# djene-mengistu/UAPS

Hardware: AMD Instinct MI355X
Metric: training images/sec (labeled+unlabeled) NEU-Seg 256x256 K=3 (higher is better)
Workload: dtype f32

## Files before the change

include/uaps_hip.h:

```cpp
#ifndef UAPS_HIP_H
#define UAPS_HIP_H

#include <stddef.h>
#include <stdint.h>

#ifdef __cplusplus
extern "C" {
#endif

typedef void* uaps_stream_t;

#define UAPS_MAX_HEADS 8
#define UAPS_MAX_CLASSES 8

#define UAPS_OK 0
#define UAPS_EINVAL (-1)
#define UAPS_ERANGE (-2)
#define UAPS_EWORKSPACE (-3)
#define UAPS_ENOFORM (-4)

int uaps_abi_version(void);
const char* uaps_error_string(int code);


// ... 81 lines not shown
                        uint8_t* keep_out, uaps_stream_t stream);
int uaps_feat_mask_apply(const float* x, const uint8_t* keep, float scale, float* y, long n, uaps_stream_t stream);

int uaps_feat_dropout_workspace_bytes(int B, int C, int H, int W, size_t* out_host);
int uaps_feat_dropout_fwd(const float* x, float* y, int B, int C, int H, int W, float u, uint8_t* keep,
                          void* workspace, size_t workspace_bytes, uaps_stream_t stream);
int uaps_feat_dropout_bwd(const float* dy, const uint8_t* keep, float* dx, int B, int C, int H, int W,
                          uaps_stream_t stream);

int uaps_sum_tensors(const float* const* in_host, int n, float* out, long count, uaps_stream_t stream);
int uaps_fanin_perturbed(const float* const* g_host, const int* mode_host, const uint8_t* const* keep_host,
                         const uint64_t* offsets_host, int n, int groups, uint64_t seed, float range, float p, int B,
                         int C, int H, int W, float* out, uaps_stream_t stream);

int uaps_feat_dropout_stats(const float* x, int B, int C, int H, int W, void* workspace, size_t workspace_bytes,
                            uaps_stream_t stream);
int uaps_fanout_perturbed(const float* f, float* const* out_host, const int* mode_host, uint8_t* const* keep_host,
                          const uint64_t* offsets_host, const float* u_host, const void* fdrop_workspace, int n, int groups,
                          uint64_t seed, float range, float p, int B, int C, int H, int W, uaps_stream_t stream);

int uaps_maxpool2x2_fwd(const float* x, int B, int C, int H, int W, float* out, uint8_t* idx, uaps_stream_t stream);


int uaps_bn_workspace_bytes(int B, int C, int H, int W, size_t* out_host);
int uaps_bn_act_fwd_train(const float* y, const float* conv_bias, const float* gamma, const float* beta,
                          float* running_mean, float* running_var, int64_t* num_batches_tracked, float momentum,
                          float eps, float slope, float drop_p, uint64_t seed, uint64_t offset, int B, int C,
                          int H, int W, float* out, float* save_mean, float* save_invstd, void* workspace,
                          size_t workspace_bytes, uaps_stream_t stream);
int uaps_bn_act_fwd_train_grouped(const float* y, const float* conv_bias, const float* gamma, const float* beta,
                                  float* running_mean, float* running_var, int64_t* num_batches_tracked, float momentum,
                                  float eps, float slope, float drop_p, uint64_t seed, uint64_t offset, int B, int C,
                                  int H, int W, int groups, float* out, float* save_mean, float* save_invstd,
                                  void* workspace, size_t workspace_bytes, uaps_stream_t stream);
int uaps_bn_act_fwd_train_partials(const void* partials, int parts_per_image, const float* y, const float* conv_bias,
                                   const float* gamma, const float* beta, float* running_mean, float* running_var,
                                   int64_t* num_batches_tracked, float momentum, float eps, float slope, float drop_p,
                                   uint64_t seed, uint64_t offset, int B, int C, int H, int W, int groups, float* out,
                                   float* save_mean, float* save_invstd, void* workspace, size_t workspace_bytes,
                                   uaps_stream_t stream);
int uaps_bn_act_bwd_grouped(const float* dout, const float* y, const float* gamma, const float* beta,
                            const float* save_mean, const float* save_invstd, float slope, float drop_p, uint64_t seed,
                            uint64_t offset, int B, int C, int H, int W, int groups, float* dy, float* dgamma,
                            float* dbeta, void* workspace, size_t workspace_bytes, uaps_stream_t stream);
int uaps_bn_act_bwd_grouped_bias(const float* dout, const float* y, const float* gamma, const float* beta,
                                 const float* save_mean, const float* save_invstd, float slope, float drop_p,
                                 uint64_t seed, uint64_t offset, int B, int C, int H, int W, int groups, float* dy,
                                 float* dgamma, float* dbeta, float* dconv_bias, void* workspace, size_t workspace_bytes,
                                 uaps_stream_t stream);
int uaps_bn_act_fwd_eval(const float* y, const float* conv_bias, const float* gamma, const float* beta,
                         const float* running_mean, const float* running_var, float eps, float slope, int B,
                         int C, int H, int W, float* out, float* save_mean, void* workspace,
                         size_t workspace_bytes, uaps_stream_t stream);
int uaps_bn_act_bwd(const float* dout, const float* y, const float* gamma, const float* beta,
                    const float* save_mean, const float* save_invstd, float slope, float drop_p, uint64_t seed,
                    uint64_t offset, int B, int C, int H, int W, float* dy, float* dgamma, float* dbeta,
                    void* workspace, size_t workspace_bytes, uaps_stream_t stream);
int uaps_bn_act_bwd_eval(const float* dout, const float* y, const float* gamma, const float* beta,
                         const float* mean_eff, const float* running_var, float eps, float slope, int B, int C,
                         int H, int W, float* dy, void* workspace, size_t workspace_bytes, uaps_stream_t stream);

int uaps_up_cat_fwd(const float* skip, const float* low, float* out, int B, int Cs, int Cl, int h, int w,
                    uaps_stream_t stream);
int uaps_up_cat_bwd(const float* dout, float* dskip, float* dlow, int B, int Cs, int Cl, int h, int w,
                    uaps_stream_t stream);

int uaps_bn_param_bounds(const float* const* gamma_host, const float* const* beta_host, const int* C_host, int n, float* out,
                         uaps_stream_t stream);

int uaps_conv_set_mode(int mode);
#define UAPS_TUNE_NO_SPLIT_FWD 1u
#define UAPS_TUNE_NO_SPLIT_WRW 2u
#define UAPS_TUNE_NO_SMALL 4u
#define UAPS_TUNE_NO_HP16 8u
#define UAPS_TUNE_WRW_ROW_MAJOR 16u
#define UAPS_TUNE_WRW_SHORT_TILES 32u
#define UAPS_TUNE_NO_TALL_FWD 64u
#define UAPS_TUNE_NO_ROW16 128u
#define UAPS_TUNE_NO_ROW_WRW 256u
#define UAPS_TUNE_DEEP_ROWS 512u
#define UAPS_TUNE_G1_NARROW 1024u
#define UAPS_TUNE_NO_G 2048u
#define UAPS_TUNE_G_DEEP 4096u
int uaps_conv_set_tuning(unsigned flags);
unsigned uaps_conv_get_tuning(void);

#define UAPS_ERR_CONV_NONFINITE 1u
#define UAPS_ERR_WRW_NONFINITE 2u
int uaps_set_error_word(unsigned* device_word);

#define UAPS_BOUND_SLOTS 16
#define UAPS_BOUND_STRIDE 64
#define UAPS_BOUND_FLOATS (UAPS_BOUND_SLOTS * UAPS_BOUND_STRIDE)
typedef struct uaps_call_hints {
    unsigned struct_size;
    const float* bound[3];
    float mul[3];
    float* out_amax;
    const float* stats_mean;
    const float* stats_bias;
    const float* residual;
    const float* dyt_y;
    const float* dyt_coef;
    float* dyt_out;
    float dyt_slope;
    int dyt_groups;
    const float* bsum_y;
    const float* bsum_mean;
    const float* bsum_invstd;
    const float* bsum_gamma;
    const float* bsum_beta;
    void* bsum_partials;
    float* bsum_max;
    float bsum_slope;
    int bsum_groups;
} uaps_call_hints;
int uaps_next_call_hints(const uaps_call_hints* hints);
int uaps_next_launch_events(void* start, void* stop);
int uaps_account(int enable);
double uaps_accounted_bytes(void);
int uaps_zero_bounds(float* bounds, long n, uaps_stream_t stream);
int uaps_conv_get_mode(void);
int uaps_conv_pack_floats(int Cout, int Cin, int ks, size_t* fwd_floats_host, size_t* bwd_floats_host);
int uaps_conv_pack_weights(const float* w, int Cout, int Cin, int ks, float* wf, float* wb, uaps_stream_t stream);
int uaps_conv_pack_weights_batch(const float* const* w_host, float* const* wf_host, float* const* wb_host,
                                 const int* Cout_host, const int* Cin_host, const int* ks_host, int n,
                                 uaps_stream_t stream);
int uaps_conv_fwd(const float* x, const float* wf, const float* bias, float* y, int B, int Cin, int Cout, int H,
                  int W, int ks, int cfg, uaps_stream_t stream);
int uaps_conv_fwd_stats(const float* x, const float* wf, const float* bias, float* y, void* stats, int B, int Cin,
                        int Cout, int H, int W, int ks, int cfg, uaps_stream_t stream);
int uaps_conv_fwd_stats_parts(int B, int Cin, int Cout, int H, int W, int ks, int cfg, int* parts_per_image_host);
int uaps_conv_bwd_data(const float* dy, const float* wb, float* dx, int B, int Cin, int Cout, int H, int W,
                       int ks, int cfg, uaps_stream_t stream);
int uaps_conv_wrw_workspace_bytes(int B, int Cin, int Cout, int H, int W, int ks, int cfg, size_t* out_host);
int uaps_conv_bwd_weight_partial(const float* dy, const float* x, int want_bias, int B, int Cin, int Cout, int H, int W,
                                 int ks, int cfg, void* workspace, size_t workspace_bytes, uaps_stream_t stream);
int uaps_conv_bwd_weight_reduce(const void* workspace, float* dw, float* dbias, int B, int Cin, int Cout, int H, int W,
                                int ks, int cfg, uaps_stream_t stream);
typedef struct uaps_wrw_reduce_item {
    const void* workspace; float* dw; float* dbias;
    int B, Cin, Cout, H, W, ks, cfg;
} uaps_wrw_reduce_item;
int uaps_conv_bwd_weight_reduce_batch(const uaps_wrw_reduce_item* items, int n, uaps_stream_t stream);
#define UAPS_CONV_X2_UP2 (1 << 10)
#define UAPS_CONV_BOUNDED (1 << 11)
int uaps_conv_fwd_cat(const float* x1, int C1, const float* x2, int C2, const float* wf, const float* bias, float* y,
                      void* stats_or_null, int B, int Cout, int H, int W, int ks, int cfg, uaps_stream_t stream);
int uaps_conv_bwd_data_cat(const float* dy, const float* wb, float* dx1, int C1, float* dx2, int C2, int B, int Cout,
                           int H, int W, int ks, int cfg, uaps_stream_t stream);
int uaps_conv_bwd_weight_partial_cat(const float* dy, const float* x1, int C1, const float* x2, int C2, int want_bias,
                                     int B, int Cout, int H, int W, int ks, int cfg, void* workspace,
                                     size_t workspace_bytes, uaps_stream_t stream);
int uaps_bn_finalize_train(const void* partials, int parts_per_image, const float* conv_bias, const float* gamma,
                           const float* beta, float* running_mean, float* running_var, int64_t* num_batches_tracked,
                           float momentum, float eps, int B, int C, int H, int W, int groups, float* save_mean,
                           float* save_invstd, void* xf, uaps_stream_t stream);
int uaps_conv_fwd_bn(const float* x_raw, const void* xf, float slope, int groups, const float* wf, const float* bias,
                     float* y, void* stats_or_null, int B, int Cin, int Cout, int H, int W, int ks, int cfg,
                     uaps_stream_t stream);
int uaps_conv_bwd_weight_partial_bn(const float* dy, const float* x_raw, const void* xf, float slope, int groups,
                                    int want_bias, int B, int Cin, int Cout, int H, int W, int ks, int cfg,
                                    void* workspace, size_t workspace_bytes, uaps_stream_t stream);
#define UAPS_CONV_FWD 0
#define UAPS_CONV_BWD_DATA 1
#define UAPS_CONV_BWD_WEIGHT 2
// ... 165 lines not shown
```

uaps_amd/_lib.py:

```python
from __future__ import annotations

import ctypes as C
import os
import subprocess
import threading

from . import config

_HERE = os.path.dirname(os.path.abspath(__file__))
LIB_PATH = config.text("UAPS_HIP_LIB") or os.path.join(_HERE, "lib", "libuaps_hip.so")
CSRC = os.path.join(_HERE, "csrc")

_lock = threading.Lock()
_tls = threading.local()
_lib = None

c_float_p = C.POINTER(C.c_float)
c_void_p = C.c_void_p

_PTR = C.c_void_p
SIGNATURES = {
    "uaps_abi_version": (C.c_int, []),
    "uaps_error_string": (C.c_char_p, [C.c_int]),
    "uaps_loss_workspace_bytes": (C.c_int, [C.c_int] * 5 + [C.POINTER(C.c_size_t)]),
# ... 79 lines not shown
    "uaps_softmax_klmap_bwd": (C.c_int, [_PTR] * 3 + [C.c_int] * 4 + [_PTR] * 3),
    "uaps_softmax_pair_fwd": (C.c_int, [_PTR, _PTR] + [C.c_int] * 5 + [_PTR, _PTR, _PTR, _PTR, C.c_size_t, _PTR]),
    "uaps_softmax_mse_bwd": (C.c_int, [_PTR] * 3 + [C.c_int] * 4 + [_PTR, _PTR]),
    "uaps_softmax_kl_bwd": (C.c_int, [_PTR] * 3 + [C.c_int] * 4 + [_PTR, _PTR]),
    "uaps_entropy_map": (C.c_int, [_PTR] + [C.c_int] * 4 + [_PTR, _PTR, _PTR, C.c_size_t, _PTR]),
    "uaps_fanin_perturbed": (C.c_int, [_PTR] * 4 + [C.c_int, C.c_int, C.c_uint64, C.c_float, C.c_float] + [C.c_int] * 4 + [_PTR, _PTR]),
    "uaps_maxpool2x2_fwd": (C.c_int, [_PTR] + [C.c_int] * 4 + [_PTR, _PTR, _PTR]),
    "uaps_adam_step": (C.c_int, [_PTR] * 5 + [C.c_int] + [C.c_double] * 5 + [C.c_long, _PTR]),
    "uaps_add_relu": (C.c_int, [_PTR, _PTR, _PTR, C.c_long, _PTR]),
    "uaps_relu_bwd": (C.c_int, [_PTR, _PTR, _PTR, C.c_long, _PTR]),
    "uaps_relu_bwd_sum": (C.c_int, [_PTR, C.c_int, _PTR, _PTR, C.c_long, _PTR]),
    "uaps_cat2": (C.c_int, [_PTR, _PTR, _PTR, C.c_long, _PTR]),
    "uaps_bn_act_bwd_prepare": (C.c_int, [_PTR] * 6 + [C.c_float] + [C.c_int] * 5 + [_PTR] * 6 + [C.c_size_t, _PTR]),
    "uaps_bn_act_bwd_apply": (C.c_int, [_PTR] * 3 + [C.c_float] + [C.c_int] * 5 + [_PTR, _PTR]),
    "uaps_bn_act_bwd_finalize": (C.c_int, [_PTR, C.c_int] + [_PTR] * 5 + [C.c_int] * 5 + [_PTR] * 6),
    "uaps_seg_confusion": (C.c_int, [_PTR, _PTR] + [C.c_int] * 4 + [_PTR, _PTR]),
    "uaps_ema_update": (C.c_int, [_PTR] * 3 + [C.c_int, C.c_float, C.c_float, _PTR]),
    "uaps_teacher_noise": (C.c_int, [_PTR] + [C.c_int] * 5 + [C.c_uint64, C.c_uint64, _PTR, _PTR]),
    "uaps_teacher_noise_apply": (C.c_int, [_PTR, _PTR] + [C.c_int] * 5 + [_PTR, _PTR]),
    "uaps_mc_consistency_workspace_bytes": (C.c_int, [C.POINTER(C.c_size_t)]),
    "uaps_mc_consistency_fwd": (C.c_int, [_PTR] * 3 + [C.c_int] * 5 + [C.c_float] + [_PTR] * 4 + [C.c_size_t, _PTR]),
    "uaps_mc_consistency_bwd": (C.c_int, [_PTR] * 5 + [C.c_int] * 4 + [_PTR, _PTR]),
    "uaps_cct_dct_workspace_bytes": (C.c_int, [C.POINTER(C.c_size_t)]),
    "uaps_cct_consistency_fwd": (C.c_int, [_PTR] + [C.c_int] * 6 + [_PTR, _PTR, C.c_size_t, _PTR]),
    "uaps_cct_consistency_bwd": (C.c_int, [_PTR] + [C.c_int] * 6 + [_PTR, _PTR, _PTR]),
    "uaps_rot90_batch": (C.c_int, [_PTR, _PTR] + [C.c_int] * 5 + [_PTR, _PTR, _PTR]),
    "uaps_rot_consistency_fwd": (C.c_int, [_PTR, C.c_int, _PTR] + [C.c_int] * 6 + [_PTR, _PTR, C.c_size_t, _PTR]),
    "uaps_rot_consistency_bwd": (C.c_int, [_PTR, C.c_int, _PTR] + [C.c_int] * 6 + [_PTR, _PTR, _PTR, _PTR]),
    "uaps_cps_workspace_bytes": (C.c_int, [C.c_int] * 5 + [C.POINTER(C.c_size_t)]),
    "uaps_cps_fwd": (C.c_int, [_PTR] * 3 + [C.c_int] * 5 + [C.c_float] + [_PTR] * 4 + [C.c_size_t, _PTR]),
    "uaps_cps_bwd": (C.c_int, [_PTR] * 7 + [C.c_int] * 5 + [_PTR] * 3),
}


HINTED = ("uaps_conv_fwd", "uaps_conv_fwd_stats", "uaps_conv_fwd_bn", "uaps_conv_fwd_cat", "uaps_conv_bwd_data", "uaps_conv_bwd_data_cat",
          "uaps_conv_bwd_weight_partial", "uaps_conv_bwd_weight_partial_bn", "uaps_conv_bwd_weight_partial_cat",
          "uaps_bn_act_fwd_train_partials", "uaps_bn_finalize_train", "uaps_bn_act_bwd_grouped", "uaps_bn_act_bwd_grouped_bias",
          "uaps_bn_act_bwd_apply", "uaps_up_cat_fwd", "uaps_cat2", "uaps_add_relu", "uaps_pairloss_bwd", "uaps_rot90_batch")
for _n in HINTED:
    SIGNATURES[_n + "_h"] = (SIGNATURES[_n][0], [_PTR] + list(SIGNATURES[_n][1]))
del _n


class UapsHipError(RuntimeError):
    pass


def build(verbose: bool = False, jobs: int = 8) -> str:
    cmd = ["make", "-C", CSRC, f"-j{jobs}"]
    r = subprocess.run(cmd, stdout=subprocess.PIPE, stderr=subprocess.STDOUT, text=True)
    if verbose or r.returncode != 0:
        print(r.stdout)
    if r.returncode != 0:
        raise UapsHipError("building libuaps_hip.so failed (see output above)")
    return LIB_PATH


def lib() -> C.CDLL:
    global _lib
    if _lib is not None:
        return _lib
    with _lock:
        if _lib is None:
            if not os.path.exists(LIB_PATH):
                raise UapsHipError(
                    f"{LIB_PATH} not found: the UAPS HIP kernels are not built. Run "
                    "`make -C uaps_amd/csrc` (needs hipcc; cross-compiles for gfx950 without a GPU). "
                    "uaps_amd has no CPU or PyTorch fallback for these ops.")
            l = C.CDLL(LIB_PATH)
            for name, (res, args) in SIGNATURES.items():
                try:
                    fn = getattr(l, name)
                except AttributeError as e:
                    raise UapsHipError(f"libuaps_hip.so does not export {name}; rebuild it") from e
                fn.restype, fn.argtypes = res, args
            _configure_from_environment(l)
            _lib = l
    return _lib


_TUNE_ENV = (("UAPS_DIAG_NO_SPLIT_FWD", 1, None), ("UAPS_DIAG_NO_SPLIT_WRW", 2, None), ("UAPS_DIAG_NO_SMALL", 4, None),
             ("UAPS_DIAG_NO_HP16", 8, None), ("UAPS_SWRW_COLMAJOR", 16, "0"), ("UAPS_WRW_TALL", 32, "0"), ("UAPS_FWD_TALL", 64, "0"),
             ("UAPS_DIAG_NO_ROW16", 128, None), ("UAPS_DIAG_NO_ROW_WRW", 256, None), ("UAPS_DIAG_DEEP_ROWS", 512, None),
             ("UAPS_DIAG_G1_NARROW", 1024, None), ("UAPS_DIAG_NO_G", 2048, None), ("UAPS_DIAG_G_DEEP", 4096, None))


def _configure_from_environment(l) -> None:
    mode = config.text("UAPS_CONV_MODE")
    if mode:
        m = 0 if mode[0] in "0ef" else (1 if mode[0] in "1bs" else 2)
        if l.uaps_conv_set_mode(m) != 0:
            raise UapsHipError(f"UAPS_CONV_MODE={mode}: uaps_conv_set_mode failed")
    flags = 0
    for name, bit, on_value in _TUNE_ENV:
        v = config.text(name)
        if v is not None and (on_value is None or v == on_value):
            flags |= bit
    l.uaps_conv_set_tuning(flags)


class quiet_gc:

    def __enter__(self):
        import gc
        gc.collect()
        self.was = gc.isenabled()
        gc.disable()
        return self

    def __exit__(self, *exc):
        import gc
        if self.was:
            gc.enable()
        return False


class WrwReduceItem(C.Structure):
    _fields_ = [("workspace", C.c_void_p), ("dw", C.c_void_p), ("dbias", C.c_void_p), ("B", C.c_int), ("Cin", C.c_int), ("Cout", C.c_int),
                ("H", C.c_int), ("W", C.c_int), ("ks", C.c_int), ("cfg", C.c_int)]


class CallHints(C.Structure):
    _fields_ = [("struct_size", C.c_uint), ("bound", C.c_void_p * 3), ("mul", C.c_float * 3), ("out_amax", C.c_void_p),
                ("stats_mean", C.c_void_p), ("stats_bias", C.c_void_p), ("residual", C.c_void_p),
                ("dyt_y", C.c_void_p), ("dyt_coef", C.c_void_p), ("dyt_out", C.c_void_p), ("dyt_slope", C.c_float), ("dyt_groups", C.c_int),
                ("bsum_y", C.c_void_p), ("bsum_mean", C.c_void_p), ("bsum_invstd", C.c_void_p), ("bsum_gamma", C.c_void_p),
                ("bsum_beta", C.c_void_p), ("bsum_partials", C.c_void_p), ("bsum_max", C.c_void_p), ("bsum_slope", C.c_float),
                ("bsum_groups", C.c_int)]


class ConvCall(C.Structure):
    _fields_ = [("struct_size", C.c_uint), ("op", C.c_int), ("B", C.c_int), ("Cin", C.c_int), ("Cout", C.c_int), ("H", C.c_int),
                ("W", C.c_int), ("ks", C.c_int), ("cfg", C.c_int), ("x", C.c_void_p), ("C1", C.c_int), ("x2", C.c_void_p),
                ("w_packed", C.c_void_p), ("bias", C.c_void_p), ("y", C.c_void_p), ("y2", C.c_void_p), ("y_grad", C.c_void_p),
                ("stats", C.c_void_p), ("xf", C.c_void_p), ("xf_slope", C.c_float), ("xf_groups", C.c_int), ("want_bias", C.c_int),
                ("workspace", C.c_void_p), ("workspace_bytes", C.c_size_t), ("stream", C.c_void_p), ("hints", CallHints)]


def mk_hints(bounds=(), out_amax=None, stats=None, residual=None, dyt=None, bsum=None):
    h = getattr(_tls, "hints", None)
    if h is None:
        h = _tls.hints = CallHints()
        h.struct_size = C.sizeof(CallHints)
    for i in range(3):
        h.bound[i] = None
    h.out_amax = h.stats_mean = h.stats_bias = None
    h.residual = residual.data_ptr() if residual is not None else None
    if dyt is not None:
        h.dyt_y, h.dyt_coef, h.dyt_out, h.dyt_slope, h.dyt_groups = dyt[0].data_ptr(), dyt[1].data_ptr(), dyt[2].data_ptr(), float(dyt[3]), int(dyt[4])
    else:
        h.dyt_y = h.dyt_coef = h.dyt_out = None
        h.dyt_slope, h.dyt_groups = 0.0, 0
    if bsum is not None:
        (h.bsum_y, h.bsum_mean, h.bsum_invstd, h.bsum_gamma, h.bsum_beta, h.bsum_partials, h.bsum_max) = [t.data_ptr() for t in bsum[:7]]
        h.bsum_slope, h.bsum_groups = float(bsum[7]), int(bsum[8])
    else:
        h.bsum_y = h.bsum_mean = h.bsum_invstd = h.bsum_gamma = h.bsum_beta = h.bsum_partials = h.bsum_max = None
        h.bsum_slope, h.bsum_groups = 0.0, 0
    if stats is not None:
        if stats[0] is not None:
            h.stats_mean = stats[0].data_ptr()
        if stats[1] is not None:
            h.stats_bias = stats[1].data_ptr()
    for i, b in enumerate(bounds):
        if b is not None:
            h.bound[i], h.mul[i] = b[0].data_ptr(), float(b[1])
    if out_amax is not None:
# ... 103 lines not shown
```

uaps_amd/config.py:

```python
from __future__ import annotations

import os
from typing import Dict

_seen: Dict[str, tuple] = {}

DOC = {
    "UAPS_HIP_LIB": "path of another build of libuaps_hip.so with the same ABI (same-box A/B of two kernel builds)",
    "UAPS_CONV_MODE": "arithmetic of the convolutions: 2 / h16 (default), 1 / split (exact three-piece bf16), 0 / exact (fp32 MFMA)",
    "UAPS_DEFER_WRW_REDUCE": "weight-gradient reductions batched behind the backward (conv.deferred_reduces)",
    "UAPS_EARLY_WRW_REDUCE": "... and the decoders' share of them on a side stream beside the encoder's backward",
    "UAPS_EARLY_ADAM": "the decoders' Adam step behind their early reductions (world size 1)",
    "UAPS_FUSED_UP2": "bilinear x2 formed in the staging of up4's first convolution instead of materialised",
    "UAPS_FUSED_BN_SUMS": "BatchNorm-backward sums in the epilogue of the 16 -> 16 input-gradient row kernel (measured a wash: off)",
    "UAPS_LAZY_BN_BWD": "BatchNorm backward in two halves on the 256-wide decoder layers (lazybn)",
    "UAPS_PAIR_CFG": "cfg bits of the pair-loss kernels (diagnosis)",
    "UAPS_FUSED_FANOUT": "all perturbed copies of a feature map written by one pass over it",
    "UAPS_EPILOGUE_STATS": "BatchNorm statistics in the producing convolution's epilogue",
    "UAPS_VIRTUAL_CAT": "two-source convolutions instead of a materialised torch.cat in the UpBlocks",
    "UAPS_FUSED_FAN": "perturbation backward fused into the gradient fan-in kernel",
    "UAPS_DECODER_CHAINS": "decoders are dealt round-robin onto this many streams (diagnosis)",
    "UAPS_FAN_BESIDE": "perturbed feature copies written on a side stream beside the encoder's next levels",
    "UAPS_PACK_BESIDE": "the decoders' weights packed on a side stream beside the encoder's forward",
    "UAPS_FUSED_POOL": "2x2 max-pool fused into the fan-out / fan-in kernels",
    "UAPS_FUSED_BN_CONV": "BatchNorm + LeakyReLU applied in the consuming convolution's staging",
    "UAPS_DECODER_STREAMS": "one HIP stream per auxiliary decoder (bench.py switches it on for the headline)",
    "UAPS_STAT_SHIFT": "BatchNorm partial sums formed about running_mean - conv bias",
    "UAPS_INPUT_IN_GRAPH": "the captured step reads the batch from its own static input buffers (filled by the concatenation kernel)",
}


def _raw(name: str):
    return os.environ.get(name)


def flag(name: str, default: bool) -> bool:
    v = _raw(name)
    val = default if v is None or v == "" else (v != "0")
    _seen[name] = (default, val)
    return val


def integer(name: str, default: int) -> int:
    v = _raw(name)
    val = default if v is None or v == "" else int(v)
    _seen[name] = (default, val)
    return val


def text(name: str, default=None):
    v = _raw(name)
    val = default if v is None or v == "" else v
    _seen[name] = (default, val)
    return val


def non_default() -> Dict[str, object]:
    out = {k: v for k, (d, v) in sorted(_seen.items()) if v != d}
    for k in sorted(os.environ):
        if k.startswith("UAPS_") and k not in _seen:
            out[k] = os.environ[k]
    return out
```

uaps_amd/csrc/resample.hip:

```cpp
#include <hip/hip_runtime.h>
#include <stdint.h>
#include "../../include/uaps_hip.h"
#include "hints.hpp"
#include "rn_math.hpp"

namespace {
using uaps::mul_rn;
constexpr int kThreads = 256;
inline int grid_for(long work, int cap = 4096) {
    long b = (work + kThreads - 1) / kThreads;
    if (b > cap) b = cap;
    return (int)(b < 1 ? 1 : b);
}
inline bool al16(const void* p) { return (reinterpret_cast<uintptr_t>(p) & 15) == 0; }

__device__ __forceinline__ float lerp2(float a0, float v0, float a1, float v1) { return __builtin_fmaf(a1, v1, mul_rn(a0, v0)); }

__device__ __forceinline__ float bilerp(const float* __restrict__ p, int w, int h0, int h1, float lh0, float lh1, int w0, int w1,
                                        float lw0, float lw1) {
    const float top = lerp2(lw0, p[(long)h0 * w + w0], lw1, p[(long)h0 * w + w1]);
    const float bot = lerp2(lw0, p[(long)h1 * w + w0], lw1, p[(long)h1 * w + w1]);
    return lerp2(lh0, top, lh1, bot);
}

template <bool VEC>
__global__ __launch_bounds__(kThreads) void up_cat_fwd_kernel(const float* __restrict__ skip, const float* __restrict__ low,
                                                              float* __restrict__ out, int B, int Cs, int Cl, int h, int w,
                                                              float rh, float rw) {
    const int H = 2 * h, W = 2 * w;
    const int Ct = Cs + Cl;
    constexpr int V = VEC ? 4 : 1;
    const long Wg = W / V;
    const long total = (long)B * Ct * H * Wg;
    for (long g = (long)blockIdx.x * kThreads + threadIdx.x; g < total; g += (long)gridDim.x * kThreads) {
        const int xg = (int)(g % Wg);
        long t = g / Wg;
        const int oy = (int)(t % H); t /= H;
        const int c = (int)(t % Ct);
        const int b = (int)(t / Ct);
        const long o = (((long)b * Ct + c) * H + oy) * W + (long)xg * V;
        if (c < Cs) {
            const long si = (((long)b * Cs + c) * H + oy) * W + (long)xg * V;
            if (VEC) *reinterpret_cast<float4*>(out + o) = *reinterpret_cast<const float4*>(skip + si);
            else out[o] = skip[si];
        } else {
            const float* p = low + ((long)b * Cl + (c - Cs)) * h * w;
            const float sy = mul_rn(rh, (float)oy);
            const int h0 = (int)sy, h1 = h0 + (h0 < h - 1 ? 1 : 0);
            const float lh1 = sy - h0, lh0 = 1.f - lh1;
            float v[V];
#pragma unroll
            for (int k = 0; k < V; ++k) {
                const int ox = xg * V + k;
                const float sx = mul_rn(rw, (float)ox);
                const int w0 = (int)sx, w1 = w0 + (w0 < w - 1 ? 1 : 0);
                const float lw1 = sx - w0, lw0 = 1.f - lw1;
                v[k] = bilerp(p, w, h0, h1, lh0, lh1, w0, w1, lw0, lw1);
            }
            if (VEC) *reinterpret_cast<float4*>(out + o) = make_float4(v[0], v[1], v[2], v[3]);
            else out[o] = v[0];
        }
    }
}

template <int TC, int RPT>
__global__ __launch_bounds__(kThreads) void up2x_tiled_kernel(const float* __restrict__ low, float* __restrict__ out, int h, int w,
                                                              float rh, float rw, int tiles_x, int tiles_y, float* __restrict__ amax_out) {
    constexpr int TG = 1024 / TC, TR = TG * RPT, LR = TR / 2 + 2, LC = TC / 2 + 2, LCP = LC + 1;
    __shared__ float sL[LR * LCP];
    const int H = 2 * h, W = 2 * w;
    int bid = blockIdx.x;
    const int tx = bid % tiles_x; bid /= tiles_x;
    const int ty = bid % tiles_y;
    const long plane = bid / tiles_y;
    const int oy0 = ty * TR, ox0 = tx * TC;
    const int sy0 = (int)mul_rn(rh, (float)oy0), sx0 = (int)mul_rn(rw, (float)ox0);
    const float* p = low + plane * h * w;
    for (int u = threadIdx.x; u < LR * LC; u += kThreads) {
        const int r = u / LC, cidx = u % LC;
        const int yy = sy0 + r, xx = sx0 + cidx;
        sL[r * LCP + cidx] = (yy < h && xx < w) ? p[(long)yy * w + xx] : 0.f;
    }
    __syncthreads();
    const int xg = threadIdx.x % (TC / 4), row = threadIdx.x / (TC / 4);
    const int ox = ox0 + xg * 4;
    float am = 0.f;
    int w0[4], w1[4];
    float lw0[4], lw1[4];
#pragma unroll
    for (int k = 0; k < 4; ++k) {
        const float sx = mul_rn(rw, (float)(ox + k));
        w0[k] = (int)sx; w1[k] = w0[k] + (w0[k] < w - 1 ? 1 : 0);
        lw1[k] = sx - w0[k]; lw0[k] = 1.f - lw1[k];
    }
#pragma unroll
    for (int i = 0; i < RPT; ++i) {
    const int oy = oy0 + row + i * TG;
    if (oy < H && ox < W) {
    const float sy = mul_rn(rh, (float)oy);
    const int h0 = (int)sy, h1 = h0 + (h0 < h - 1 ? 1 : 0);
    const float lh1 = sy - h0, lh0 = 1.f - lh1;
    const float* r0 = &sL[(h0 - sy0) * LCP - sx0];
    const float* r1 = &sL[(h1 - sy0) * LCP - sx0];
    float v[4];
#pragma unroll
    for (int k = 0; k < 4; ++k) {
        const float top = lerp2(lw0[k], r0[w0[k]], lw1[k], r0[w1[k]]);
        const float bot = lerp2(lw0[k], r1[w0[k]], lw1[k], r1[w1[k]]);
        v[k] = lerp2(lh0, top, lh1, bot);
    }
    *reinterpret_cast<float4*>(out + (plane * H + oy) * W + ox) = make_float4(v[0], v[1], v[2], v[3]);
    am = fmaxf(am, fmaxf(fmaxf(fabsf(v[0]), fabsf(v[1])), fmaxf(fabsf(v[2]), fabsf(v[3]))));
    }
    }
    if (amax_out) {
        __shared__ float sm[16];
        uaps::block_amax_to(amax_out, am, sm);
    }
}

constexpr int kLx = 32, kPc = 2 * kLx + 8;

__device__ __forceinline__ float tap_weight(float r, int o, int n_out, int n_in, int i) {
    if (o < 0 || o >= n_out) return 0.f;
    const float sx = mul_rn(r, (float)o);
    const int i0 = (int)sx, i1 = i0 + (i0 < n_in - 1 ? 1 : 0);
    const float l1 = sx - i0, l0 = 1.f - l1;
    return (i0 == i ? l0 : 0.f) + (i1 == i ? l1 : 0.f);
}

template <int kLy>
__global__ __launch_bounds__(kThreads) void up_cat_bwd_low_kernel(const float* __restrict__ dout, float* __restrict__ dlow, int B,
                                                                  int Cs, int Cl, int h, int w, float rh, float rw,
                                                                  int tiles_x, int tiles_y) {
    constexpr int kPr = 2 * kLy + 6;
    __shared__ __attribute__((aligned(16))) float sA[kPr * kPc];
    __shared__ float sT[kPr * kLx];
    __shared__ float sWx[kLx][7], sWy[kLy][7];
    const int H = 2 * h, W = 2 * w, Ct = Cs + Cl;
    int bid = blockIdx.x;
    const int tx = bid % tiles_x; bid /= tiles_x;
    const int ty = bid % tiles_y; bid /= tiles_y;
    const int c = bid % Cl, b = bid / Cl;
    const int iy0 = ty * kLy, ix0 = tx * kLx;
    const int oy0 = 2 * iy0 - 3, ox0 = 2 * ix0 - 4;
    const float* p = dout + (((long)b * Ct + Cs + c) * H) * W;
    const bool vec = (W % 4) == 0;
    for (int u = threadIdx.x; u < kPr * (kPc / 4); u += kThreads) {
        const int r = u / (kPc / 4), x4 = (u % (kPc / 4)) * 4;
        const int oy = oy0 + r, ox = ox0 + x4;
        float4 v = make_float4(0.f, 0.f, 0.f, 0.f);
        if (oy >= 0 && oy < H) {
            if (vec && ox >= 0 && ox + 3 < W) {
                v = *reinterpret_cast<const float4*>(p + (long)oy * W + ox);
            } else {
                const float* q = p + (long)oy * W;
                if (ox >= 0 && ox < W) v.x = q[ox];
                if (ox + 1 >= 0 && ox + 1 < W) v.y = q[ox + 1];
                if (ox + 2 >= 0 && ox + 2 < W) v.z = q[ox + 2];
                if (ox + 3 >= 0 && ox + 3 < W) v.w = q[ox + 3];
            }
        }
        *reinterpret_cast<float4*>(&sA[r * kPc + x4]) = v;
    }
    if (threadIdx.x < kLx * 7) {
        const int l = threadIdx.x / 7, k = threadIdx.x % 7;
        sWx[l][k] = tap_weight(rw, 2 * (ix0 + l) - 3 + k, W, w, ix0 + l);
    }
    if (threadIdx.x < kLy * 7) {
        const int l = threadIdx.x / 7, k = threadIdx.x % 7;
        sWy[l][k] = tap_weight(rh, 2 * (iy0 + l) - 3 + k, H, h, iy0 + l);
    }
    const int lx = threadIdx.x % kLx, ly0 = threadIdx.x / kLx;
    const int ix = ix0 + lx;
    __syncthreads();
    float wx[7];
#pragma unroll
    for (int k = 0; k < 7; ++k) wx[k] = sWx[lx][k];
    for (int r = ly0; r < kPr; r += kThreads / kLx) {
        const float2* a2 = reinterpret_cast<const float2*>(&sA[r * kPc + 2 * lx]);
        const float2 p0 = a2[0], p1 = a2[1], p2 = a2[2], p3 = a2[3];
        const float a[7] = {p0.y, p1.x, p1.y, p2.x, p2.y, p3.x, p3.y};
        float row = 0.f;
#pragma unroll
        for (int k = 0; k < 7; ++k) row += wx[k] * a[k];
        sT[r * kLx + lx] = row;
    }
    __syncthreads();
#pragma unroll
    for (int j = 0; j < kLy / 8; ++j) {
        const int ly = ly0 + 8 * j, iy = iy0 + ly;
        if (ix < w && iy < h) {
            float acc = 0.f;
#pragma unroll
            for (int k = 0; k < 7; ++k) acc += sWy[ly][k] * sT[(2 * ly + k) * kLx + lx];
            dlow[(((long)b * Cl + c) * h + iy) * w + ix] = acc;
        }
    }
}

template <bool VEC>
__global__ __launch_bounds__(kThreads) void slice_channels_kernel(const float* __restrict__ src, float* __restrict__ dst, int B,
                                                                  int Ct, int c0, int Cn, long HW) {
    constexpr int V = VEC ? 4 : 1;
    const long per = HW / V;
    const long total = (long)B * Cn * per;
    for (long g = (long)blockIdx.x * kThreads + threadIdx.x; g < total; g += (long)gridDim.x * kThreads) {
        const long i = g % per;
        const long t = g / per;
        const int c = (int)(t % Cn);
        const int b = (int)(t / Cn);
        const long s = (((long)b * Ct + c0 + c) * HW) + i * V, d = (((long)b * Cn + c) * HW) + i * V;
        if (VEC) *reinterpret_cast<float4*>(dst + d) = *reinterpret_cast<const float4*>(src + s);
        else dst[d] = src[s];
    }
}
}

static int up_cat_fwd_impl(float* amax_out, const float* skip, const float* low, float* out, int B, int Cs, int Cl, int h, int w, uaps_stream_t stream);
extern "C" int uaps_up_cat_fwd(const float* skip, const float* low, float* out, int B, int Cs, int Cl, int h, int w,
                               uaps_stream_t stream) {
    return up_cat_fwd_impl(uaps::take_hints().out_amax, skip, low, out, B, Cs, Cl, h, w, stream);
}
extern "C" int uaps_up_cat_fwd_h(const uaps_call_hints* hints, const float* skip, const float* low, float* out, int B, int Cs, int Cl, int h,
                                 int w, uaps_stream_t stream) {
    UAPS_READ_HINTS(hints, hh);
    return up_cat_fwd_impl(hh.out_amax, skip, low, out, B, Cs, Cl, h, w, stream);
}
static int up_cat_fwd_impl(float* amax_out, const float* skip, const float* low, float* out, int B, int Cs, int Cl, int h, int w, uaps_stream_t stream) {
    if (!skip || !low || !out || B <= 0 || Cs < 0 || Cl <= 0 || h <= 0 || w <= 0) return UAPS_EINVAL;
    const int H = 2 * h, W = 2 * w;
    const float rh = H > 1 ? (float)(h - 1) / (float)(H - 1) : 0.f, rw = W > 1 ? (float)(w - 1) / (float)(W - 1) : 0.f;
    hipStream_t s = (hipStream_t)stream;
    const long total = (long)B * (Cs + Cl) * H * W;
    uaps::account_bytes(4.0 * ((double)B * Cl * h * w + 2.0 * B * Cs * H * W + (double)B * Cl * H * W));
    if (amax_out && !(Cs == 0 && W % 4 == 0 && al16(out))) return UAPS_ERANGE;
    if (Cs == 0 && W % 4 == 0 && al16(out)) {
        const bool wide = W >= 64, tall = wide && H >= 64;
        const int TC = wide ? 64 : 32, TR = (1024 / TC) * (tall ? 4 : 1);
        const int tiles_x = (W + TC - 1) / TC, tiles_y = (H + TR - 1) / TR;
        const long nblk = (long)B * Cl * tiles_x * tiles_y;
        if (nblk > 0x7fffffffL) return UAPS_ERANGE;
        if (tall) hipLaunchKernelGGL((up2x_tiled_kernel<64, 4>), dim3((unsigned)nblk), dim3(kThreads), 0, s, low, out, h, w, rh, rw, tiles_x, tiles_y, amax_out);
        else if (wide) hipLaunchKernelGGL((up2x_tiled_kernel<64, 1>), dim3((unsigned)nblk), dim3(kThreads), 0, s, low, out, h, w, rh, rw, tiles_x, tiles_y, amax_out);
        else hipLaunchKernelGGL((up2x_tiled_kernel<32, 1>), dim3((unsigned)nblk), dim3(kThreads), 0, s, low, out, h, w, rh, rw, tiles_x, tiles_y, amax_out);
        return (int)hipGetLastError();
    }
    if (W % 4 == 0 && al16(skip) && al16(out))
        hipLaunchKernelGGL(up_cat_fwd_kernel<true>, dim3(grid_for(total / 4)), dim3(kThreads), 0, s, skip, low, out, B, Cs, Cl, h, w, rh, rw);
    else
        hipLaunchKernelGGL(up_cat_fwd_kernel<false>, dim3(grid_for(total)), dim3(kThreads), 0, s, skip, low, out, B, Cs, Cl, h, w, rh, rw);
    return (int)hipGetLastError();
}

extern "C" int uaps_up_cat_bwd(const float* dout, float* dskip, float* dlow, int B, int Cs, int Cl, int h, int w,
                               uaps_stream_t stream) {
    if (!dout || !dlow || B <= 0 || Cs < 0 || Cl <= 0 || h <= 0 || w <= 0) return UAPS_EINVAL;
    const int H = 2 * h, W = 2 * w;
    const float rh = H > 1 ? (float)(h - 1) / (float)(H - 1) : 0.f, rw = W > 1 ? (float)(w - 1) / (float)(W - 1) : 0.f;
    hipStream_t s = (hipStream_t)stream;
    uaps::account_bytes(4.0 * ((double)B * Cl * H * W + (double)B * Cl * h * w + (dskip ? 2.0 * B * Cs * H * W : 0.0)));
    if (dskip && Cs > 0) {
        const long HW = (long)H * W;
        if (HW % 4 == 0 && al16(dout) && al16(dskip))
            hipLaunchKernelGGL(slice_channels_kernel<true>, dim3(grid_for((long)B * Cs * HW / 4)), dim3(kThreads), 0, s, dout, dskip, B, Cs + Cl, 0, Cs, HW);
        else
            hipLaunchKernelGGL(slice_channels_kernel<false>, dim3(grid_for((long)B * Cs * HW)), dim3(kThreads), 0, s, dout, dskip, B, Cs + Cl, 0, Cs, HW);
    }
    const int ly = h >= 32 ? 32 : 8;
    const int tiles_x = (w + kLx - 1) / kLx, tiles_y = (h + ly - 1) / ly;
    const long nblk = (long)B * Cl * tiles_x * tiles_y;
    if (nblk > 0x7fffffffL) return UAPS_ERANGE;
    if (ly == 32) hipLaunchKernelGGL(up_cat_bwd_low_kernel<32>, dim3((unsigned)nblk), dim3(kThreads), 0, s, dout, dlow, B, Cs, Cl, h, w, rh, rw, tiles_x, tiles_y);
    else hipLaunchKernelGGL(up_cat_bwd_low_kernel<8>, dim3((unsigned)nblk), dim3(kThreads), 0, s, dout, dlow, B, Cs, Cl, h, w, rh, rw, tiles_x, tiles_y);
    return (int)hipGetLastError();
}
```

Before: 2670.

## Stream bilinear x2 gradient fold over row bands with register-rotated vertical accumulation

Adds a band-streaming kernel for the low-resolution gradient of the bilinear x2 upsample. Each 64-thread workgroup walks a band of rows, double-buffering eight output rows at a time in shared memory with prefetch into registers. It folds each row horizontally, then accumulates the vertical taps in three rotating registers, so every dout row is read once instead of re-staged per 32x32 tile. The new path is the default when W%4==0 and dout is 16-byte aligned, and a tuning bit restores the old kernel. Both kernels now use explicit mul/add rounding helpers so their results match, at the cost of a new file, new launch heuristics and narrow workgroups.

Result: no change. 2689 (median of 6 runs) (+0.7%).

```diff
diff --git a/include/uaps_hip.h b/include/uaps_hip.h
--- a/include/uaps_hip.h
+++ b/include/uaps_hip.h
@@ -187,6 +187,7 @@
 #define UAPS_TUNE_G1_NARROW 1024u
 #define UAPS_TUNE_NO_G 2048u
 #define UAPS_TUNE_G_DEEP 4096u
+#define UAPS_TUNE_NO_UP_ROWS (UAPS_TUNE_G_DEEP << 1)
 int uaps_conv_set_tuning(unsigned flags);
 unsigned uaps_conv_get_tuning(void);
 
diff --git a/uaps_amd/_lib.py b/uaps_amd/_lib.py
--- a/uaps_amd/_lib.py
+++ b/uaps_amd/_lib.py
@@ -185,7 +185,8 @@
 _TUNE_ENV = (("UAPS_DIAG_NO_SPLIT_FWD", 1, None), ("UAPS_DIAG_NO_SPLIT_WRW", 2, None), ("UAPS_DIAG_NO_SMALL", 4, None),
              ("UAPS_DIAG_NO_HP16", 8, None), ("UAPS_SWRW_COLMAJOR", 16, "0"), ("UAPS_WRW_TALL", 32, "0"), ("UAPS_FWD_TALL", 64, "0"),
              ("UAPS_DIAG_NO_ROW16", 128, None), ("UAPS_DIAG_NO_ROW_WRW", 256, None), ("UAPS_DIAG_DEEP_ROWS", 512, None),
-             ("UAPS_DIAG_G1_NARROW", 1024, None), ("UAPS_DIAG_NO_G", 2048, None), ("UAPS_DIAG_G_DEEP", 4096, None))
+             ("UAPS_DIAG_G1_NARROW", 1024, None), ("UAPS_DIAG_NO_G", 2048, None), ("UAPS_DIAG_G_DEEP", 4096, None),
+             ("UAPS_DIAG_NO_UP_ROWS", 8192, None))
 
 
 def _configure_from_environment(l) -> None:
diff --git a/uaps_amd/config.py b/uaps_amd/config.py
--- a/uaps_amd/config.py
+++ b/uaps_amd/config.py
@@ -26,6 +26,7 @@
     "UAPS_FUSED_BN_CONV": "BatchNorm + LeakyReLU applied in the consuming convolution's staging",
     "UAPS_DECODER_STREAMS": "one HIP stream per auxiliary decoder (bench.py switches it on for the headline)",
     "UAPS_STAT_SHIFT": "BatchNorm partial sums formed about running_mean - conv bias",
+    "UAPS_DIAG_NO_UP_ROWS": "the bilinear x2 gradient fold on the 32-column tile kernels instead of the band-streaming form (A/B; default: band-streaming)",
     "UAPS_INPUT_IN_GRAPH": "the captured step reads the batch from its own static input buffers (filled by the concatenation kernel)",
 }
 
diff --git a/uaps_amd/csrc/resample.hip b/uaps_amd/csrc/resample.hip
--- a/uaps_amd/csrc/resample.hip
+++ b/uaps_amd/csrc/resample.hip
@@ -3,9 +3,13 @@
 #include "../../include/uaps_hip.h"
 #include "hints.hpp"
 #include "rn_math.hpp"
+#include "resample_taps.hpp"
 
 namespace {
 using uaps::mul_rn;
+using uaps::tap_first;
+using uaps::tap_next;
+using uaps::tap_weight;
 constexpr int kThreads = 256;
 inline int grid_for(long work, int cap = 4096) {
     long b = (work + kThreads - 1) / kThreads;
@@ -120,14 +124,6 @@
 }
 
 constexpr int kLx = 32, kPc = 2 * kLx + 8;
-
-__device__ __forceinline__ float tap_weight(float r, int o, int n_out, int n_in, int i) {
-    if (o < 0 || o >= n_out) return 0.f;
-    const float sx = mul_rn(r, (float)o);
-    const int i0 = (int)sx, i1 = i0 + (i0 < n_in - 1 ? 1 : 0);
-    const float l1 = sx - i0, l0 = 1.f - l1;
-    return (i0 == i ? l0 : 0.f) + (i1 == i ? l1 : 0.f);
-}
 
 template <int kLy>
 __global__ __launch_bounds__(kThreads) void up_cat_bwd_low_kernel(const float* __restrict__ dout, float* __restrict__ dlow, int B,
@@ -181,9 +177,9 @@
         const float2* a2 = reinterpret_cast<const float2*>(&sA[r * kPc + 2 * lx]);
         const float2 p0 = a2[0], p1 = a2[1], p2 = a2[2], p3 = a2[3];
         const float a[7] = {p0.y, p1.x, p1.y, p2.x, p2.y, p3.x, p3.y};
-        float row = 0.f;
-#pragma unroll
-        for (int k = 0; k < 7; ++k) row += wx[k] * a[k];
+        float row = tap_first(wx[0], a[0]);
+#pragma unroll
+        for (int k = 1; k < 7; ++k) row = tap_next(row, wx[k], a[k]);
         sT[r * kLx + lx] = row;
     }
     __syncthreads();
@@ -191,9 +187,9 @@
     for (int j = 0; j < kLy / 8; ++j) {
         const int ly = ly0 + 8 * j, iy = iy0 + ly;
         if (ix < w && iy < h) {
-            float acc = 0.f;
-#pragma unroll
-            for (int k = 0; k < 7; ++k) acc += sWy[ly][k] * sT[(2 * ly + k) * kLx + lx];
+            float acc = tap_first(sWy[ly][0], sT[(2 * ly) * kLx + lx]);
+#pragma unroll
+            for (int k = 1; k < 7; ++k) acc = tap_next(acc, sWy[ly][k], sT[(2 * ly + k) * kLx + lx]);
             dlow[(((long)b * Cl + c) * h + iy) * w + ix] = acc;
         }
     }
@@ -267,6 +263,8 @@
         else
             hipLaunchKernelGGL(slice_channels_kernel<false>, dim3(grid_for((long)B * Cs * HW)), dim3(kThreads), 0, s, dout, dskip, B, Cs + Cl, 0, Cs, HW);
     }
+    if (W % 4 == 0 && al16(dout) && !(uaps_conv_get_tuning() & UAPS_TUNE_NO_UP_ROWS))
+        return uaps::up_fold_rows(dout, dlow, B, Cs, Cl, h, w, rh, rw, s);
     const int ly = h >= 32 ? 32 : 8;
     const int tiles_x = (w + kLx - 1) / kLx, tiles_y = (h + ly - 1) / ly;
     const long nblk = (long)B * Cl * tiles_x * tiles_y;
diff --git a/uaps_amd/csrc/resample_rows.hip b/uaps_amd/csrc/resample_rows.hip
--- /dev/null
+++ b/uaps_amd/csrc/resample_rows.hip
@@ -0,0 +1,148 @@
+#include <hip/hip_runtime.h>
+#include <stdint.h>
+#include "../../include/uaps_hip.h"
+#include "resample_taps.hpp"
+
+namespace {
+using uaps::tap_first;
+using uaps::tap_next;
+using uaps::tap_weight;
+
+#ifndef UAPS_FOLD_BAND
+#define UAPS_FOLD_BAND 64
+#endif
+constexpr int kRowT = 64, kRowR = 8, kRowBand = UAPS_FOLD_BAND, kRowPairs = (kRowBand + 3 + 3) & ~3;
+static_assert(kRowBand >= 4 && kRowBand <= 64, "the pair table is sized for bands of at most 64 rows");
+
+__device__ __forceinline__ float fold_x(const float* __restrict__ s, const float (&wx)[7]) {
+    const float2* a2 = reinterpret_cast<const float2*>(s);
+    const float2 p0 = a2[0], p1 = a2[1], p2 = a2[2], p3 = a2[3];
+    const float a[7] = {p0.y, p1.x, p1.y, p2.x, p2.y, p3.x, p3.y};
+    float row = tap_first(wx[0], a[0]);
+#pragma unroll
+    for (int k = 1; k < 7; ++k) row = tap_next(row, wx[k], a[k]);
+    return row;
+}
+
+typedef float f4 __attribute__((ext_vector_type(4)));
+
+template <int TW, bool HALO>
+__global__ __launch_bounds__(kRowT) void up_fold_rows_kernel(const float* __restrict__ dout, float* __restrict__ dlow, int Cs, int Cl,
+                                                             int h, int w, float rh, float rw, int nseg, int bands, int bh, int ncu) {
+    constexpr int G = kRowT / TW, RS = 2 * TW + 8, L4 = TW / 2, NL = G * kRowR * L4 / kRowT;
+    static_assert(!HALO || G == 1, "segments with a halo are one per workgroup");
+    __shared__ __attribute__((aligned(16))) float sA[2][G * kRowR * RS];
+    __shared__ __attribute__((aligned(16))) float sP[kRowPairs * 8];
+    const int H = 2 * h, W = 2 * w, Ct = Cs + Cl, t = threadIdx.x;
+    const int band = blockIdx.x % bands;
+    const int cg = blockIdx.x / bands;
+    const int iy0 = band * bh, iy1 = min(iy0 + bh, h);
+    const int npairs = (iy1 - iy0 + 3 + 3) & ~3;
+    const int oy_first = 2 * (iy0 - 2);
+    const float* src[NL];
+    int srow[NL], sdst[NL];
+#pragma unroll
+    for (int i = 0; i < NL; ++i) {
+        const int q = t + kRowT * i, gq = q / (kRowR * L4), rem = q % (kRowR * L4), r = rem / L4, c4 = rem % L4;
+        const int cu = cg * G + gq;
+        const int plane = HALO ? cu / nseg : cu, seg = HALO ? cu - plane * nseg : 0;
+        const int ox = 2 * seg * TW + 4 * c4;
+        const int b = plane / Cl, c = plane - b * Cl;
+        src[i] = (cu < ncu && ox < W) ? dout + (((long)b * Ct + Cs + c) * H) * W + ox : nullptr;
+        srow[i] = r;
+        sdst[i] = (gq * kRowR + r) * RS + 4 + 4 * c4;
+    }
+    const int g = t / TW, lx = t % TW;
+    const int cu = cg * G + g;
+    const int plane = HALO ? cu / nseg : cu, seg = HALO ? cu - plane * nseg : 0;
+    const int ix = seg * TW + lx;
+    const bool mine = cu < ncu && ix < w;
+    float wx[7];
+#pragma unroll
+    for (int k = 0; k < 7; ++k) wx[k] = tap_weight(rw, 2 * ix - 3 + k, W, w, ix);
+    const float* hsrc = nullptr;
+    int hdst = 0;
+    if (HALO) {
+        const int r = t >> 1, side = t & 1, ox = side ? 2 * seg * TW + 2 * TW : 2 * seg * TW - 4;
+        if (t < 2 * kRowR && cu < ncu && ox >= 0 && ox < W) {
+            const int b = plane / Cl, c = plane - b * Cl;
+            hsrc = dout + (((long)b * Ct + Cs + c) * H) * W + ox;
+        }
+        hdst = r * RS + (side ? 4 + 2 * TW : 0);
+    } else {
+        for (int u = t; u < 2 * G * kRowR * 2; u += kRowT) {
+            const int side = u & 1, r = u >> 1;
+            *reinterpret_cast<float4*>(&sA[0][r * RS + (side ? 4 + 2 * TW : 0)]) = make_float4(0.f, 0.f, 0.f, 0.f);
+        }
+    }
+    for (int u = t; u < npairs * 8; u += kRowT) {
+        const int j = iy0 - 2 + (u >> 3), k = u & 7;
+        const int iy = j + (k < 3 ? k - 1 : (k < 6 ? k - 4 : 2)), tap = k < 3 ? 5 - 2 * k : (k < 6 ? 12 - 2 * k : 0);
+        sP[u] = (k < 7 && iy >= 0 && iy < h) ? tap_weight(rh, 2 * iy - 3 + tap, H, h, iy) : 0.f;
+    }
+    const f4 zero4 = {0.f, 0.f, 0.f, 0.f};
+    f4 v[NL], hv = zero4;
+#pragma unroll
+    for (int i = 0; i < NL; ++i) {
+        const int oy = oy_first + srow[i];
+        v[i] = (src[i] && oy >= 0 && oy < H) ? *reinterpret_cast<const f4*>(src[i] + (long)oy * W) : zero4;
+    }
+    if (HALO && t < 2 * kRowR) {
+        const int oy = oy_first + (t >> 1);
+        hv = (hsrc && oy >= 0 && oy < H) ? *reinterpret_cast<const f4*>(hsrc + (long)oy * W) : zero4;
+    }
+    float a0 = 0.f, a1 = 0.f, a2 = 0.f, a3 = 0.f;
+    float* orow = dlow + ((long)plane * h + (iy0 - 3)) * w + ix;
+    const int nst = npairs / (kRowR / 2);
+    for (int st = 0; st < nst; ++st) {
+        float* buf = sA[st & 1];
+#pragma unroll
+        for (int i = 0; i < NL; ++i) *reinterpret_cast<f4*>(&buf[sdst[i]]) = v[i];
+        if (HALO && t < 2 * kRowR) *reinterpret_cast<f4*>(&buf[hdst]) = hv;
+        __syncthreads();
+        if (st + 1 < nst) {
+            const int oyb = oy_first + kRowR * (st + 1);
+#pragma unroll
+            for (int i = 0; i < NL; ++i) {
+                const int oy = oyb + srow[i];
+                v[i] = (src[i] && oy >= 0 && oy < H) ? *reinterpret_cast<const f4*>(src[i] + (long)oy * W) : zero4;
+            }
+            if (HALO && t < 2 * kRowR) {
+                const int oy = oyb + (t >> 1);
+                hv = (hsrc && oy >= 0 && oy < H) ? *reinterpret_cast<const f4*>(hsrc + (long)oy * W) : zero4;
+            }
+        }
+        const float* rows = buf + g * kRowR * RS + 2 * lx;
+#pragma unroll
+        for (int pr = 0; pr < kRowR / 2; ++pr) {
+            const int jm1 = iy0 - 3 + st * (kRowR / 2) + pr;
+            const float te = fold_x(rows + (2 * pr) * RS, wx), to = fold_x(rows + (2 * pr + 1) * RS, wx);
+            const float4 pa = *reinterpret_cast<const float4*>(&sP[(st * (kRowR / 2) + pr) * 8]);
+            const float4 pb = *reinterpret_cast<const float4*>(&sP[(st * (kRowR / 2) + pr) * 8 + 4]);
+            a0 = tap_next(a0, pa.x, te); a1 = tap_next(a1, pa.y, te); a2 = tap_next(a2, pa.z, te);
+            a0 = tap_next(a0, pa.w, to); a1 = tap_next(a1, pb.x, to); a2 = tap_next(a2, pb.y, to);
+            a3 = tap_first(pb.z, to);
+            if (mine && jm1 >= iy0 && jm1 < iy1) *orow = a0;
+            orow += w;
+            a0 = a1; a1 = a2; a2 = a3;
+        }
+    }
+}
+}
+
+int uaps::up_fold_rows(const float* dout, float* dlow, int B, int Cs, int Cl, int h, int w, float rh, float rw, hipStream_t s) {
+    const int tw = w <= 16 ? 16 : (w <= 32 ? 32 : 64);
+    const int nseg = (w + tw - 1) / tw;
+    const long ncu = (long)B * Cl * nseg, ngrp = (ncu + kRowT / tw - 1) / (kRowT / tw);
+    int bh = kRowBand;
+    while (bh > 16 && ngrp * ((h + bh - 1) / bh) < 2048) bh /= 2;
+    const int bands = (h + bh - 1) / bh;
+    const long nblk = ngrp * bands;
+    if (nblk > 0x7fffffffL || ncu + kRowT > 0x7fffffffL) return UAPS_ERANGE;
+    const dim3 grid((unsigned)nblk), blk(kRowT);
+    if (tw == 16) hipLaunchKernelGGL((up_fold_rows_kernel<16, false>), grid, blk, 0, s, dout, dlow, Cs, Cl, h, w, rh, rw, nseg, bands, bh, (int)ncu);
+    else if (tw == 32) hipLaunchKernelGGL((up_fold_rows_kernel<32, false>), grid, blk, 0, s, dout, dlow, Cs, Cl, h, w, rh, rw, nseg, bands, bh, (int)ncu);
+    else if (nseg == 1) hipLaunchKernelGGL((up_fold_rows_kernel<64, false>), grid, blk, 0, s, dout, dlow, Cs, Cl, h, w, rh, rw, nseg, bands, bh, (int)ncu);
+    else hipLaunchKernelGGL((up_fold_rows_kernel<64, true>), grid, blk, 0, s, dout, dlow, Cs, Cl, h, w, rh, rw, nseg, bands, bh, (int)ncu);
+    return (int)hipGetLastError();
+}
diff --git a/uaps_amd/csrc/resample_taps.hpp b/uaps_amd/csrc/resample_taps.hpp
--- /dev/null
+++ b/uaps_amd/csrc/resample_taps.hpp
@@ -0,0 +1,17 @@
+#pragma once
+#include <hip/hip_runtime.h>
+#include "rn_math.hpp"
+namespace uaps {
+__device__ __forceinline__ float tap_first(float w, float a) { return __builtin_fmaf(w, a, 0.f); }
+__device__ __forceinline__ float tap_next(float acc, float w, float a) { return add_rn(acc, mul_rn(w, a)); }
+
+__device__ __forceinline__ float tap_weight(float r, int o, int n_out, int n_in, int i) {
+    if (o < 0 || o >= n_out) return 0.f;
+    const float sx = mul_rn(r, (float)o);
+    const int i0 = (int)sx, i1 = i0 + (i0 < n_in - 1 ? 1 : 0);
+    const float l1 = sx - i0, l0 = 1.f - l1;
+    return (i0 == i ? l0 : 0.f) + (i1 == i ? l1 : 0.f);
+}
+
+int up_fold_rows(const float* dout, float* dlow, int B, int Cs, int Cl, int h, int w, float rh, float rw, hipStream_t s);
+}
```
